# revdotcom/reverb

Hardware: NVIDIA H100
Metric: rtfx_attention_rescoring_30s_chunks (higher is better)
Workload: dtype bf16

## Files before the change

reverb_b200/csrc/attention_tc.cu:

```cuda
#include <cuda.h>
#include <math.h>
#include <stdlib.h>

#include <algorithm>

#include "kernels.h"

namespace rvb {

constexpr int AT_BM = 128;
constexpr int AT_BN = 64;
constexpr int AT_DK = 64;
constexpr int AT_ST = 4;
constexpr int AT_THREADS = 288;
constexpr uint32_t AT_Q_BYTES = AT_BM * AT_DK * 2;
constexpr uint32_t AT_TILE_BYTES = AT_BN * AT_DK * 2;
constexpr uint32_t AT_SMEM_FIXED = AT_Q_BYTES + 2 * AT_ST * AT_TILE_BYTES + 256  + 1024 ;

__device__ __forceinline__ float fast_exp2(float x) {
  float y;
  asm("ex2.approx.ftz.f32 %0, %1;" : "=f"(y) : "f"(x));
  return y;
}

struct AttnTcParams {
  bf16* out;
  long long ldo;
  const float* key_bias;
  const int* k_lens;
  int Tq, Tk, H;
  int chunk;
  int left;
  const uint32_t* key_bits;
  int bits_ld;
  float scale_log2;
};

__global__ void __launch_bounds__(AT_THREADS, 1)
attention_tc_kernel(const __grid_constant__ CUtensorMap tmQ, const __grid_constant__ CUtensorMap tmK,
                    const __grid_constant__ CUtensorMap tmV, const AttnTcParams p) {
  extern __shared__ uint8_t smem_raw[];
  uint8_t* smem = reinterpret_cast<uint8_t*>((reinterpret_cast<uintptr_t>(smem_raw) + 1023) & ~uintptr_t(1023));
  uint8_t* sQ = smem;
  uint8_t* sK = sQ + AT_Q_BYTES;
  uint8_t* sV = sK + AT_ST * AT_TILE_BYTES;
  uint64_t* bars = reinterpret_cast<uint64_t*>(sV + AT_ST * AT_TILE_BYTES);
  uint64_t* q_full = bars;
  uint64_t* k_full = bars + 1;
  uint64_t* k_empty = k_full + AT_ST;
  uint64_t* v_full = k_empty + AT_ST;
  uint64_t* v_empty = v_full + AT_ST;
  static_assert(1 + 4 * AT_ST <= 32, "barrier block is 256 bytes");
  float* s_bias = reinterpret_cast<float*>(bars + 32);

  const int warp = threadIdx.x >> 5, lane = threadIdx.x & 31;
  const int qtile = blockIdx.x, h = blockIdx.y, g = blockIdx.z;
  const int q0 = qtile * AT_BM;
  int klen = p.Tk;
  if (p.k_lens) klen = min(klen, __ldg(p.k_lens + g));
  auto vis_lo = [&](int i) { return (p.chunk > 0 && p.left >= 0) ? max(0, (i / p.chunk - p.left) * p.chunk) : 0; };
  auto vis_hi = [&](int i) { return p.chunk > 0 ? min(klen, (i / p.chunk + 1) * p.chunk) : klen; };
  const int jt0 = vis_lo(q0) / AT_BN;
  const int ntiles = max(0, (vis_hi(q0 + AT_BM - 1) + AT_BN - 1) / AT_BN - jt0);
  const long long krow0 = (long long)g * p.Tk;

  if (threadIdx.x == 0) {
    mbar_init(q_full, 1);
    for (int i = 0; i < AT_ST; ++i) {
      mbar_init(&k_full[i], 1);
      mbar_init(&k_empty[i], 8);
      mbar_init(&v_full[i], 1);
      mbar_init(&v_empty[i], 8);
    }
    fence_barrier_init();
  }
  {
    const float* kb = p.key_bias ? p.key_bias + ((long long)g * p.H + h) * p.Tk : nullptr;
    for (int kk = threadIdx.x; kk < ntiles * AT_BN; kk += AT_THREADS) {
      const int key = jt0 * AT_BN + kk;
      s_bias[kk] = (key < klen) ? (kb ? __ldg(kb + key) * p.scale_log2 : 0.f) : -INFINITY;
    }
  }
  __syncthreads();

  if (warp == 8) {
    if (lane == 0 && ntiles > 0) {
      tma_prefetch_desc(&tmQ);
      tma_prefetch_desc(&tmK);
      tma_prefetch_desc(&tmV);
      mbar_expect_tx(q_full, AT_Q_BYTES);
      tma_load_2d(sQ, &tmQ, q_full, h * AT_DK, (int)((long long)g * p.Tq + q0));
      for (int n = 0; n < ntiles; ++n) {
        const int st = n % AT_ST, ph = ((n / AT_ST) & 1) ^ 1;
        const int krow = (int)(krow0 + (jt0 + n) * AT_BN);
        mbar_wait(&k_empty[st], ph);
        mbar_expect_tx(&k_full[st], AT_TILE_BYTES);
        tma_load_2d(sK + st * AT_TILE_BYTES, &tmK, &k_full[st], h * AT_DK, krow);
        mbar_wait(&v_empty[st], ph);
        mbar_expect_tx(&v_full[st], AT_TILE_BYTES);
        tma_load_2d(sV + st * AT_TILE_BYTES, &tmV, &v_full[st], h * AT_DK, krow);
      }
    }
    return;
  }

  const int wg = warp >> 2, wl = warp & 3;
  const int rloc = wg * 64 + wl * 16 + (lane >> 2);
  const int row[2] = {q0 + rloc, q0 + rloc + 8};
  const int cq = 2 * (lane & 3);
  float o[32];
#pragma unroll
  for (int i = 0; i < 32; ++i) o[i] = 0.f;
  float m_run[2] = {-INFINITY, -INFINITY}, row_sum[2] = {0.f, 0.f};
  if (ntiles > 0) mbar_wait(q_full, 0);
  const uint64_t qdesc = make_sw128_desc(smem_u32(sQ + wg * (AT_Q_BYTES / 2)));
#pragma unroll 1
  for (int j = 0; j < ntiles; ++j) {
    const int st = j % AT_ST, ph = (j / AT_ST) & 1;
    float s[32];
    mbar_wait(&k_full[st], ph);
    {
      const uint64_t kdesc = make_sw128_desc(smem_u32(sK + st * AT_TILE_BYTES));
      wgmma_fence_regs<32>(s);
      wgmma_fence();
#pragma unroll
      for (int k = 0; k < AT_DK / 16; ++k) wgmma_m64n64k16_ss(s, qdesc + 2 * k, kdesc + 2 * k, k != 0);
      wgmma_commit();
      wgmma_wait<0>();
      wgmma_fence_regs<32>(s);
    }
    if (lane == 0) mbar_arrive(&k_empty[st]);
    const int kbase = (jt0 + j) * AT_BN;
    const float* bias = s_bias + j * AT_BN;
    float tmax[2] = {-INFINITY, -INFINITY};
#pragma unroll
    for (int jj = 0; jj < 8; ++jj) {
      const float2 b2 = *reinterpret_cast<const float2*>(bias + 8 * jj + cq);
#pragma unroll
      for (int i = 0; i < 2; ++i) {
        s[4 * jj + 2 * i] = fmaf(s[4 * jj + 2 * i], p.scale_log2, b2.x);
        s[4 * jj + 2 * i + 1] = fmaf(s[4 * jj + 2 * i + 1], p.scale_log2, b2.y);
      }
    }
    if (p.chunk > 0) {
#pragma unroll
      for (int i = 0; i < 2; ++i) {
        const int lo = vis_lo(row[i]) - kbase, hi = vis_hi(row[i]) - kbase;
#pragma unroll
        for (int jj = 0; jj < 8; ++jj)
#pragma unroll
          for (int c = 0; c < 2; ++c) {
            const int col = 8 * jj + cq + c;
            if (col < lo || col >= hi) s[4 * jj + 2 * i + c] = -INFINITY;
          }
      }
    }
    if (p.key_bits) {
#pragma unroll
      for (int i = 0; i < 2; ++i) {
        const uint32_t* mw = p.key_bits + ((long long)g * p.Tq + min(row[i], p.Tq - 1)) * p.bits_ld + (kbase >> 5);
        const uint32_t w0 = __ldg(mw), w1 = __ldg(mw + 1);
#pragma unroll
        for (int jj = 0; jj < 8; ++jj)
#pragma unroll
          for (int c = 0; c < 2; ++c) {
            const int col = 8 * jj + cq + c;
            const uint32_t word = (col < 32) ? w0 : w1;
            if (!((word >> (col & 31)) & 1u)) s[4 * jj + 2 * i + c] = -INFINITY;
          }
      }
    }
#pragma unroll
    for (int jj = 0; jj < 8; ++jj)
#pragma unroll
      for (int i = 0; i < 2; ++i) tmax[i] = fmaxf(tmax[i], fmaxf(s[4 * jj + 2 * i], s[4 * jj + 2 * i + 1]));
#pragma unroll
    for (int i = 0; i < 2; ++i) {
      tmax[i] = fmaxf(tmax[i], __shfl_xor_sync(0xffffffffu, tmax[i], 1));
      tmax[i] = fmaxf(tmax[i], __shfl_xor_sync(0xffffffffu, tmax[i], 2));
    }
    float m_eff[2];
#pragma unroll
    for (int i = 0; i < 2; ++i) {
      const float m_new = fmaxf(m_run[i], tmax[i]);
      const float f = (m_new == -INFINITY || m_run[i] == m_new) ? 1.f : fast_exp2(m_run[i] - m_new);
      m_run[i] = m_new;
      row_sum[i] *= f;
#pragma unroll
      for (int jj = 0; jj < 8; ++jj) {
        o[4 * jj + 2 * i] *= f;
        o[4 * jj + 2 * i + 1] *= f;
      }
      m_eff[i] = (m_new == -INFINITY) ? 0.f : m_new;
    }
    uint32_t pa[16];
#pragma unroll
    for (int jj = 0; jj < 8; ++jj)
#pragma unroll
      for (int i = 0; i < 2; ++i) {
        const uint32_t w = pack_bf16x2(fast_exp2(s[4 * jj + 2 * i] - m_eff[i]), fast_exp2(s[4 * jj + 2 * i + 1] - m_eff[i]));
        const float2 pr = unpack_bf16x2(w);
        row_sum[i] += pr.x + pr.y;
        pa[2 * jj + i] = w;
      }
    mbar_wait(&v_full[st], ph);
    {
      const uint64_t vdesc = make_sw128_desc(smem_u32(sV + st * AT_TILE_BYTES));
      wgmma_fence_regs<32>(o);
      wgmma_fence();
#pragma unroll
      for (int ks = 0; ks < AT_BN / 16; ++ks)
        wgmma_m64n64k16_rs_tb(o, pa + 4 * ks, vdesc + (uint64_t)((ks * 16 * 128) >> 4));
      wgmma_commit();
      wgmma_wait<0>();
      wgmma_fence_regs<32>(o);
    }
    if (lane == 0) mbar_arrive(&v_empty[st]);
  }
#pragma unroll
  for (int i = 0; i < 2; ++i) {
    float sum = row_sum[i];
    sum += __shfl_xor_sync(0xffffffffu, sum, 1);
    sum += __shfl_xor_sync(0xffffffffu, sum, 2);
    const float inv = sum > 0.f ? 1.f / sum : 0.f;
    if (row[i] < p.Tq) {
      bf16* orow = p.out + ((long long)g * p.Tq + row[i]) * p.ldo + h * AT_DK;
#pragma unroll
      for (int jj = 0; jj < 8; ++jj)
        *reinterpret_cast<uint32_t*>(orow + 8 * jj + cq) = pack_bf16x2(o[4 * jj + 2 * i] * inv, o[4 * jj + 2 * i + 1] * inv);
    }
  }
}

__global__ void __launch_bounds__(256)
relpos_prep_kernel(const bf16* __restrict__ k, long long ldk, const bf16* __restrict__ pos, long long ldp,
                   const float* __restrict__ bias_u, const float* __restrict__ bias_v, bf16* __restrict__ kpp,
                   float* __restrict__ cbias, int B, int T, int H, int dk) {
  const long long row = ((long long)blockIdx.x * blockDim.x + threadIdx.x) >> 5;
  const int lane = threadIdx.x & 31;
  if (row >= (long long)B * T) return;
  const int b = (int)(row / T), t = (int)(row - (long long)b * T);
  const int d = H * dk;
  const bf16* kr = k + row * ldk;
  const bf16* pr = pos + (long long)t * ldp;
  bf16* orow = kpp + row * d;
  for (int h = 0; h < H; ++h) {
    float acc = 0.f;
    for (int c = 2 * lane; c < dk; c += 64) {
      const int col = h * dk + c;
      float2 kv = unpack_bf16x2(*reinterpret_cast<const uint32_t*>(kr + col));
      float2 pv = unpack_bf16x2(*reinterpret_cast<const uint32_t*>(pr + col));
// ... 56 lines not shown
                       ((reinterpret_cast<uintptr_t>(pos) & 15) == 0) && ((reinterpret_cast<uintptr_t>(kpp) & 15) == 0) &&
                       ((reinterpret_cast<uintptr_t>(bias_u) & 15) == 0) && ((reinterpret_cast<uintptr_t>(bias_v) & 15) == 0);
  if (aligned && dk == 64)
    relpos_prep_vec_kernel<8><<<grid, 256, 0, stream>>>(k, ldk, pos, ldp, bias_u, bias_v, kpp, cbias, B, T, H);
  else if (aligned && dk == 128)
    relpos_prep_vec_kernel<16><<<grid, 256, 0, stream>>>(k, ldk, pos, ldp, bias_u, bias_v, kpp, cbias, B, T, H);
  else if (aligned && dk == 32)
    relpos_prep_vec_kernel<4><<<grid, 256, 0, stream>>>(k, ldk, pos, ldp, bias_u, bias_v, kpp, cbias, B, T, H);
  else
    relpos_prep_kernel<<<grid, 256, 0, stream>>>(k, ldk, pos, ldp, bias_u, bias_v, kpp, cbias, B, T, H, dk);
  RVB_COUNT_LAUNCH();
  RVB_CHECK_LAUNCH();
  return 0;
}

typedef CUresult (*EncodeTiledFn)(CUtensorMap*, CUtensorMapDataType, cuuint32_t, void*, const cuuint64_t*,
                                  const cuuint64_t*, const cuuint32_t*, const cuuint32_t*, CUtensorMapInterleave,
                                  CUtensorMapSwizzle, CUtensorMapL2promotion, CUtensorMapFloatOOBfill);
static EncodeTiledFn g_encode_att = nullptr;

static int tmap_2d(CUtensorMap* m, const void* base, long long cols, long long rows, long long ld_elems,
                   int box_rows) {
  cuuint64_t dims[2] = {(cuuint64_t)cols, (cuuint64_t)rows};
  cuuint64_t str[1] = {(cuuint64_t)ld_elems * 2};
  cuuint32_t box[2] = {64, (cuuint32_t)box_rows};
  cuuint32_t estr[2] = {1, 1};
  CUresult r = g_encode_att(m, CU_TENSOR_MAP_DATA_TYPE_BFLOAT16, 2, const_cast<void*>(base), dims, str, box, estr,
                            CU_TENSOR_MAP_INTERLEAVE_NONE, CU_TENSOR_MAP_SWIZZLE_128B, CU_TENSOR_MAP_L2_PROMOTION_L2_256B,
                            CU_TENSOR_MAP_FLOAT_OOB_FILL_NONE);
  RVB_REQUIRE(r == CUDA_SUCCESS, "attention: cuTensorMapEncodeTiled failed (%d)", (int)r);
  return 0;
}

int launch_attention_tc(const AttnTcArgs& a, cudaStream_t stream) {
  RVB_REQUIRE(a.dk == AT_DK, "attention_tc: only d_k = 64 is built");
  RVB_REQUIRE(a.ldq % 8 == 0 && a.ldk % 8 == 0 && a.ldv % 8 == 0 && a.ldo % 8 == 0, "attention_tc: ld %% 8 != 0");
  RVB_REQUIRE(((uintptr_t)a.q & 15) == 0 && ((uintptr_t)a.k & 15) == 0 && ((uintptr_t)a.v & 15) == 0 &&
                  ((uintptr_t)a.out & 15) == 0,
              "attention_tc: operands must be 16-byte aligned");
  RVB_REQUIRE((!a.causal && a.chunk <= 0) || a.Tq == a.Tk, "attention_tc: causal / chunk masks need Tq == Tk");
  RVB_REQUIRE(!(a.causal && a.chunk > 0), "attention_tc: causal and chunk mask are exclusive");
  if (a.groups <= 0 || a.Tq <= 0) return 0;
  if (g_encode_att == nullptr) {
    void* fn = nullptr;
    cudaDriverEntryPointQueryResult qres;
    RVB_CHECK_CUDA(cudaGetDriverEntryPoint("cuTensorMapEncodeTiled", &fn, cudaEnableDefault, &qres));
    RVB_REQUIRE(fn != nullptr && qres == cudaDriverEntryPointSuccess, "cuTensorMapEncodeTiled not available");
    g_encode_att = reinterpret_cast<EncodeTiledFn>(fn);
  }
  AttnTcParams p;
  p.out = a.out;
  p.ldo = a.ldo;
  p.key_bias = a.key_bias;
  p.k_lens = a.k_lens;
  p.Tq = a.Tq;
  p.Tk = a.Tk;
  p.H = a.H;
  p.chunk = a.causal ? 1 : (a.chunk > 0 ? a.chunk : 0);
  p.left = a.causal ? -1 : a.left_chunks;
  p.key_bits = a.key_bits;
  p.bits_ld = a.bits_ld;
  RVB_REQUIRE(a.key_bits == nullptr || a.bits_ld >= 2 * ((a.Tk + 63) / 64), "attention_tc: key_bits rows are too short");
  p.scale_log2 = a.scale * 1.4426950408889634f;
  CUtensorMap tmQ, tmK, tmV;
  if (tmap_2d(&tmQ, a.q, (long long)a.H * AT_DK, (long long)a.groups * a.Tq, a.ldq, AT_BM)) return -1;
  if (tmap_2d(&tmK, a.k, (long long)a.H * AT_DK, (long long)a.groups * a.Tk, a.ldk, AT_BN)) return -1;
  if (tmap_2d(&tmV, a.v, (long long)a.H * AT_DK, (long long)a.groups * a.Tk, a.ldv, AT_BN)) return -1;
  dim3 grid((a.Tq + AT_BM - 1) / AT_BM, a.H, a.groups);
  const size_t smem = AT_SMEM_FIXED + (size_t)((a.Tk + AT_BN - 1) / AT_BN) * AT_BN * sizeof(float);
  RVB_REQUIRE(smem <= 227 * 1024, "attention_tc: Tk=%d needs %zu B of shared memory", a.Tk, smem);
  static DynSmemOptIn optin;
  if (optin.ensure(attention_tc_kernel, smem)) return -1;
  attention_tc_kernel<<<grid, AT_THREADS, smem, stream>>>(tmQ, tmK, tmV, p);
  RVB_COUNT_LAUNCH();
  RVB_CHECK_LAUNCH();
  return 0;
}

}
```

include/rvb_b200.h:

```cpp
#ifndef RVB_B200_H_
#define RVB_B200_H_

#if defined(__GNUC__)
#define RVB_API __attribute__((visibility("default")))
#else
#define RVB_API
#endif

#ifdef __cplusplus
extern "C" {
#endif

typedef struct rvb_model rvb_model;

typedef struct rvb_model_config {
  int input_dim;
  int d_model;
  int heads;
  int ffn_dim;
  int num_blocks;
  int cnn_kernel;
  int causal;
  int cnn_layer_norm;
  int num_langs;
// ... 104 lines not shown

typedef struct rvb_aligner rvb_aligner;
RVB_API long long rvb_aligner_workspace_bytes(int U, int total_frames, int want_loglik);
RVB_API rvb_aligner* rvb_aligner_begin(rvb_model* m, const int* h_labels, int U, int total_frames, int V, int blank_id,
                                       int want_loglik, long long budget_bytes, void* stream);
RVB_API int rvb_aligner_push(rvb_aligner* a, const float* d_logp, int n_rows, void* stream);
RVB_API int rvb_aligner_finish(rvb_aligner* a, int* h_frames, int* h_first, int* h_last, int* h_peak, float* h_peak_logp,
                               float* h_score, double* h_loglik, void* stream);
RVB_API void rvb_aligner_abort(rvb_aligner* a);

RVB_API int rvb_gemm_bf16(const void* d_A, const void* d_W, const float* d_bias, int M, int N, int K, int act, int out_mode,
                  float alpha, void* d_out, int ldo, void* stream);
RVB_API int rvb_gemm_bf16_rows(const void* d_A, const void* d_W, const float* d_bias, int M, int N, int K, int act,
                               int out_mode, float alpha, void* d_out, int ldo, const int* d_row_lens, int rows_per_batch,
                               void* stream);
RVB_API int rvb_gemm_bf16x3(const void* d_A, const void* d_W, const float* d_bias, int M, int N, int K, int act, int out_mode,
                            float alpha, void* d_out, int ldo, void* stream);
RVB_API int rvb_f32_to_bf16_pair(const float* d_x, void* d_out, long long rows, int width, void* stream);
RVB_API long long rvb_gemm_logsoftmax_gather_ws_bytes(int M, int N);
RVB_API int rvb_gemm_logsoftmax_gather(const void* d_A, const void* d_W, const float* d_bias, int M, int N, int K,
                                       const int* d_gather, void* d_ws, float* d_out, void* stream);
RVB_API int rvb_layernorm(const float* d_x, const float* d_gamma, const float* d_beta, float eps, int M, int d,
                  void* d_out_bf16, float* d_out_f32, void* stream);
RVB_API int rvb_attention(const void* d_q, const void* d_k, const void* d_v, const void* d_p, const float* d_bias_u,
                  const float* d_bias_v, void* d_out, int ldq, int ldk, int ldv, int ldp, int ldo, int Bq, int Tq, int Tk,
                  int H, int dk, int q_per_kv, const int* d_k_lens, const int* d_q_lens, int causal, float scale,
                  void* stream);
RVB_API int rvb_attention_tc(const void* d_q, const void* d_k, const void* d_v, void* d_out, int ldq, int ldk, int ldv,
                             int ldo, int groups, int Tq, int Tk, int H, int dk, const float* d_key_bias,
                             const int* d_k_lens, int causal, float scale, void* stream);
RVB_API int rvb_attention_tc_chunked(const void* d_q, const void* d_k, const void* d_v, void* d_out, int ldq, int ldk,
                                     int ldv, int ldo, int groups, int Tq, int Tk, int H, int dk, const float* d_key_bias,
                                     const int* d_k_lens, int chunk, int left_chunks, float scale, void* stream);
RVB_API int rvb_relpos_prep(const void* d_k, int ldk, const void* d_pos, int ldp, const float* d_bias_u,
                            const float* d_bias_v, void* d_kpp, float* d_cbias, int B, int T, int H, int dk,
                            void* stream);
RVB_API int rvb_f32_to_bf16(const float* d_x, void* d_out, long long n, void* stream);

#ifdef __cplusplus
}
#endif
#endif
```

reverb_b200/_lib.py:

```python
from __future__ import annotations

import ctypes as C
import os
from typing import Optional

_HERE = os.path.dirname(os.path.abspath(__file__))
LIB_PATH = os.environ.get("RVB_LIB_PATH") or os.path.join(_HERE, "librvb_b200.so")


class ModelConfig(C.Structure):
    _fields_ = [(n, C.c_int) for n in (
        "input_dim", "d_model", "heads", "ffn_dim", "num_blocks", "cnn_kernel", "causal",
        "cnn_layer_norm", "num_langs", "vocab", "dec_heads", "dec_ffn_dim", "dec_blocks", "r_dec_blocks",
        "sos_id", "eos_id", "precision")]


class SegConfig(C.Structure):
    _fields_ = [(n, C.c_int) for n in (
        "sample_rate", "sinc_filters", "sinc_kernel", "sinc_stride", "conv_channels", "conv_kernel", "lstm_hidden",
        "lstm_layers", "linear_dim", "linear_layers", "num_classes")]


class EmbConfig(C.Structure):
    _fields_ = [("sample_rate", C.c_int), ("num_mel_bins", C.c_int), ("m_channels", C.c_int), ("embed_dim", C.c_int),
# ... 32 lines not shown
                                       _vp, _vp, _vp, _vp]),
    "rvb_search_submit": (_i, [_vp, _vp, _vp, _i, _vp, _vp, _i, _i, _i, _i, _vp]),
    "rvb_search_submit_biased": (_i, [_vp, _vp, _vp, _i, _vp, _vp, _i, _i, _i, _i, _vp, _vp]),
    "rvb_context_graph_create": (_vp, [_i, _vp, _vp, _vp, _vp, _vp, _vp, _vp, _i, _i]),
    "rvb_context_graph_destroy": (None, [_vp]),
    "rvb_ctc_prefix_beam_search_biased": (_i, [_vp, _vp, _i, _vp, _i, _i, _i, _i, _i, _vp, _vp, _vp, _vp, _vp, _vp,
                                               _vp]),
    "rvb_rescoring_submit": (_i, [_vp, _i, _vp, _i, _f, _i, _i, _vp, _vp, _vp, _vp, _vp, _vp]),
    "rvb_rescoring_collect": (_i, [_vp, _i, _vp, _vp, _vp]),
    "rvb_ticket_release": (_i, [_vp, _i]),
    "rvb_decoder_step_topk": (_i, [_vp, _vp, _vp, _i, _i, _i, _vp, _i, _vp, _i, _i, _vp, _vp, _vp]),
    "rvb_decoder_cache_begin": (_i, [_vp, _vp, _vp, _i, _i, _i, _i, _vp, _i, _vp]),
    "rvb_decoder_cache_step": (_i, [_vp, _vp, _vp, _i, _vp, _vp, _vp]),
    "rvb_decoder_cache_end": (_i, [_vp]),
    "rvb_decoder_step_logp": (_i, [_vp, _vp, _vp, _i, _i, _i, _vp, _i, _vp, _i, _vp, _vp]),
    "rvb_attention_rescoring": (_i, [_vp, _vp, _vp, _i, _i, _vp, _vp, _i, _i, _vp, _i, _f, _vp, _vp, _vp]),
    "rvb_ctc_force_align": (_i, [_vp, _i, _vp, _i, _i, _vp, _vp, _i, _i, _vp, _vp, _vp, _vp, _vp, _vp, _vp, _vp]),
    "rvb_aligner_workspace_bytes": (_ll, [_i, _i, _i]),
    "rvb_aligner_begin": (_vp, [_vp, _vp, _i, _i, _i, _i, _i, _ll, _vp]),
    "rvb_aligner_push": (_i, [_vp, _vp, _i, _vp]),
    "rvb_aligner_finish": (_i, [_vp, _vp, _vp, _vp, _vp, _vp, _vp, _vp, _vp]),
    "rvb_aligner_abort": (None, [_vp]),
    "rvb_gemm_bf16": (_i, [_vp, _vp, _vp, _i, _i, _i, _i, _i, _f, _vp, _i, _vp]),
    "rvb_gemm_bf16_rows": (_i, [_vp, _vp, _vp, _i, _i, _i, _i, _i, _f, _vp, _i, _vp, _i, _vp]),
    "rvb_gemm_bf16x3": (_i, [_vp, _vp, _vp, _i, _i, _i, _i, _i, _f, _vp, _i, _vp]),
    "rvb_f32_to_bf16_pair": (_i, [_vp, _vp, _ll, _i, _vp]),
    "rvb_gemm_logsoftmax_gather_ws_bytes": (_ll, [_i, _i]),
    "rvb_gemm_logsoftmax_gather": (_i, [_vp, _vp, _vp, _i, _i, _i, _vp, _vp, _vp, _vp]),
    "rvb_layernorm": (_i, [_vp, _vp, _vp, _f, _i, _i, _vp, _vp, _vp]),
    "rvb_attention": (_i, [_vp, _vp, _vp, _vp, _vp, _vp, _vp, _i, _i, _i, _i, _i, _i, _i, _i, _i, _i, _i, _vp, _vp,
                           _i, _f, _vp]),
    "rvb_attention_tc_chunked": (_i, [_vp, _vp, _vp, _vp, _i, _i, _i, _i, _i, _i, _i, _i, _i, _vp, _vp, _i, _i, _f, _vp]),
    "rvb_attention_tc": (_i, [_vp, _vp, _vp, _vp, _i, _i, _i, _i, _i, _i, _i, _i, _i, _vp, _vp, _i, _f, _vp]),
    "rvb_relpos_prep": (_i, [_vp, _i, _vp, _i, _vp, _vp, _vp, _vp, _i, _i, _i, _i, _vp]),
    "rvb_f32_to_bf16": (_i, [_vp, _vp, _ll, _vp]),
    "rvb_seg_create": (_vp, [C.POINTER(SegConfig)]),
    "rvb_seg_set_tensor": (_i, [_vp, C.c_char_p, _vp, _ll]),
    "rvb_seg_finalize": (_i, [_vp]),
    "rvb_seg_destroy": (None, [_vp]),
    "rvb_seg_num_frames": (_i, [_vp, _i]),
    "rvb_seg_forward": (_i, [_vp, _vp, _i, _i, _vp, _vp, _vp]),
    "rvb_emb_create": (_vp, [C.POINTER(EmbConfig)]),
    "rvb_emb_set_tensor": (_i, [_vp, C.c_char_p, _vp, _ll]),
    "rvb_emb_finalize": (_i, [_vp]),
    "rvb_emb_destroy": (None, [_vp]),
    "rvb_emb_num_frames": (_i, [_vp, _i]),
    "rvb_emb_forward": (_i, [_vp, _vp, _i, _i, _vp, _i, _i, _vp, _vp, _vp]),
}

_lib: Optional[C.CDLL] = None


def load() -> C.CDLL:
    global _lib
    if _lib is not None:
        return _lib
    if not os.path.exists(LIB_PATH):
        raise RuntimeError(
            f"{LIB_PATH} is missing: build it with `python -m reverb_b200.build` "
            "(or __graft_entry__.build()). reverb_b200 has no CPU fallback.")
    lib = C.CDLL(LIB_PATH)
    for name, (res, args) in SIGNATURES.items():
        if os.environ.get("RVB_LIB_PATH") and not hasattr(lib, name):
            continue
        fn = getattr(lib, name)
        fn.restype = res
# ... 14 lines not shown
```

reverb_b200/csrc/engine.cu:

```cuda
#include <math.h>
#include <stdarg.h>
#include <stdlib.h>
#include <string.h>

#include <atomic>
#include <map>
#include <string>
#include <vector>

#include "../../include/rvb_b200.h"
#include "kernels.h"

namespace rvb {

static thread_local char g_err[1024] = "";
std::atomic<unsigned long long> g_launch_count{0};
void set_error(const char* fmt, ...) {
  va_list ap;
  va_start(ap, fmt);
  vsnprintf(g_err, sizeof(g_err), fmt, ap);
  va_end(ap);
}
const char* last_error() { return g_err; }

// ... 2149 lines not shown
  a.q = reinterpret_cast<const rvb::bf16*>(d_q);
  a.k = reinterpret_cast<const rvb::bf16*>(d_k);
  a.v = reinterpret_cast<const rvb::bf16*>(d_v);
  a.p = reinterpret_cast<const rvb::bf16*>(d_p);
  a.bias_u = d_bias_u;
  a.bias_v = d_bias_v;
  a.out = reinterpret_cast<rvb::bf16*>(d_out);
  a.ldq = ldq; a.ldk = ldk; a.ldv = ldv; a.ldp = ldp; a.ldo = ldo;
  a.Bq = Bq; a.Tq = Tq; a.Tk = Tk; a.H = H; a.dk = dk;
  a.q_per_kv = q_per_kv;
  a.k_lens = d_k_lens; a.q_lens = d_q_lens;
  a.causal = causal;
  a.scale = scale;
  return rvb::launch_attention(a, (cudaStream_t)stream);
}

RVB_API int rvb_attention_tc(const void* d_q, const void* d_k, const void* d_v, void* d_out, int ldq, int ldk, int ldv,
                             int ldo, int groups, int Tq, int Tk, int H, int dk, const float* d_key_bias,
                             const int* d_k_lens, int causal, float scale, void* stream) {
  rvb::AttnTcArgs a;
  a.q = reinterpret_cast<const rvb::bf16*>(d_q);
  a.k = reinterpret_cast<const rvb::bf16*>(d_k);
  a.v = reinterpret_cast<const rvb::bf16*>(d_v);
  a.out = reinterpret_cast<rvb::bf16*>(d_out);
  a.ldq = ldq; a.ldk = ldk; a.ldv = ldv; a.ldo = ldo;
  a.groups = groups; a.Tq = Tq; a.Tk = Tk; a.H = H; a.dk = dk;
  a.key_bias = d_key_bias;
  a.k_lens = d_k_lens;
  a.causal = causal;
  a.scale = scale;
  return rvb::launch_attention_tc(a, (cudaStream_t)stream);
}

RVB_API int rvb_attention_tc_chunked(const void* d_q, const void* d_k, const void* d_v, void* d_out, int ldq, int ldk,
                                     int ldv, int ldo, int groups, int Tq, int Tk, int H, int dk, const float* d_key_bias,
                                     const int* d_k_lens, int chunk, int left_chunks, float scale, void* stream) {
  rvb::AttnTcArgs a;
  a.q = reinterpret_cast<const rvb::bf16*>(d_q);
  a.k = reinterpret_cast<const rvb::bf16*>(d_k);
  a.v = reinterpret_cast<const rvb::bf16*>(d_v);
  a.out = reinterpret_cast<rvb::bf16*>(d_out);
  a.ldq = ldq; a.ldk = ldk; a.ldv = ldv; a.ldo = ldo;
  a.groups = groups; a.Tq = Tq; a.Tk = Tk; a.H = H; a.dk = dk;
  a.key_bias = d_key_bias;
  a.k_lens = d_k_lens;
  a.chunk = chunk;
  a.left_chunks = left_chunks;
  a.scale = scale;
  return rvb::launch_attention_tc(a, (cudaStream_t)stream);
}

RVB_API int rvb_relpos_prep(const void* d_k, int ldk, const void* d_pos, int ldp, const float* d_bias_u,
                            const float* d_bias_v, void* d_kpp, float* d_cbias, int B, int T, int H, int dk,
                            void* stream) {
  return rvb::launch_relpos_prep(reinterpret_cast<const rvb::bf16*>(d_k), ldk, reinterpret_cast<const rvb::bf16*>(d_pos),
                                 ldp, d_bias_u, d_bias_v, reinterpret_cast<rvb::bf16*>(d_kpp), d_cbias, B, T, H, dk,
                                 (cudaStream_t)stream);
}

RVB_API int rvb_f32_to_bf16(const float* d_x, void* d_out, long long n, void* stream) {
  return rvb::launch_f32_to_bf16(d_x, reinterpret_cast<rvb::bf16*>(d_out), n, (cudaStream_t)stream);
}

}
```

reverb_b200/csrc/kernels.h:

```cpp
#pragma once
#include "common.cuh"

struct rvb_model;
struct rvb_context_graph;

namespace rvb {

int search_side_stream(::rvb_model* m, cudaStream_t* out);

enum GemmAct { ACT_NONE = 0, ACT_RELU = 1, ACT_SILU = 2, ACT_GLU = 3 };
enum GemmOut {
  OUT_BF16 = 0,
  OUT_F32 = 1,
  OUT_RESID_F32 = 2,
  OUT_LSE = 3
};
inline int lse_slabs(int N) { return ((N + 255) / 256) * 2; }

struct GemmArgs {
  const bf16* A = nullptr;
  const bf16* W = nullptr;
  int M = 0, N = 0, K = 0;
  int lda = 0;
  int ldw = 0;
// ... 70 lines not shown
  const bf16* q = nullptr;
  const bf16* k = nullptr;
  const bf16* v = nullptr;
  const bf16* p = nullptr;
  const float* bias_u = nullptr;
  const float* bias_v = nullptr;
  bf16* out = nullptr;
  int ldq = 0, ldk = 0, ldv = 0, ldp = 0, ldo = 0;
  int Bq = 0, Tq = 0, Tk = 0, H = 0, dk = 0;
  int q_per_kv = 1;
  const int* k_lens = nullptr;
  const int* q_lens = nullptr;
  int causal = 0;
  float scale = 1.0f;
};
int launch_attention(const AttnArgs& a, cudaStream_t stream);

struct AttnTcArgs {
  const bf16* q = nullptr;
  const bf16* k = nullptr;
  const bf16* v = nullptr;
  bf16* out = nullptr;
  int ldq = 0, ldk = 0, ldv = 0, ldo = 0;
  int groups = 0, Tq = 0, Tk = 0, H = 0, dk = 0;
  const float* key_bias = nullptr;
  const int* k_lens = nullptr;
  int causal = 0;
  int chunk = 0, left_chunks = -1;
  const uint32_t* key_bits = nullptr;
  int bits_ld = 0;
  float scale = 1.0f;
};
int launch_attention_tc(const AttnTcArgs& a, cudaStream_t stream);
int launch_relpos_prep(const bf16* k, int ldk, const bf16* pos, int ldp, const float* bias_u, const float* bias_v,
                       bf16* kpp, float* cbias, int B, int T, int H, int dk, cudaStream_t stream);

struct AttnF32Args {
  const bf16* q = nullptr;
  const bf16* k = nullptr;
  const bf16* v = nullptr;
  const bf16* p = nullptr;
  const float* bias_u = nullptr;
  const float* bias_v = nullptr;
  bf16* out = nullptr;
  int ldq = 0, ldk = 0, ldv = 0, ldp = 0, ldo = 0;
  int q_lo = 0, k_lo = 0, v_lo = 0, p_lo = 0, o_lo = 0;
  int groups = 0, Tq = 0, Tk = 0, H = 0, dk = 0;
  const int* k_lens = nullptr;
  int chunk = 0, left = -1;
  const int* key_list = nullptr;
  const int* key_list_len = nullptr;
  int key_list_ld = 0;
};
int launch_attention_f32(const AttnF32Args& a, cudaStream_t stream);

int launch_logsoftmax_topk(const float* logits, int ld, int M, int V, int k, float* topk_val, int* topk_idx,
                           float* logp_out , int apply_softmax, cudaStream_t stream);
int launch_ctc_greedy(const int* top1_idx, int idx_stride, const int* lens, int B, int T, int blank, int* out_tokens,
                      int* out_lens, cudaStream_t stream);
struct PrefixBeamWorkspace;
size_t prefix_beam_workspace_bytes(int B, int T, int beam);
int launch_ctc_prefix_beam(const float* topk_val, const int* topk_idx, int k, const int* lens, int B, int T, int beam,
                           int blank, void* workspace, size_t workspace_bytes, int max_len, int* out_tokens,
                           int* out_times, int* out_lens, double* out_scores, int* out_nhyp, cudaStream_t stream);
struct ContextGraphView {
  const int* off = nullptr;
// ... 36 lines not shown
```

Baseline: 11910.

## Overlap QK^T of next tile with PV of current tile in attention kernel

Measured after the change: 11990, median of 6. No clear change (+0.7%).

```diff
diff --git a/reverb_b200/csrc/attention_tc.cu b/reverb_b200/csrc/attention_tc.cu
--- a/reverb_b200/csrc/attention_tc.cu
+++ b/reverb_b200/csrc/attention_tc.cu
@@ -21,6 +21,11 @@
   float y;
   asm("ex2.approx.ftz.f32 %0, %1;" : "=f"(y) : "f"(x));
   return y;
+}
+
+__device__ __forceinline__ void keep_regs16(const uint32_t* r) {
+#pragma unroll
+  for (int i = 0; i < 16; ++i) asm volatile("" ::"r"(r[i]) : "memory");
 }
 
 struct AttnTcParams {
@@ -64,7 +69,8 @@
   const int ntiles = max(0, (vis_hi(q0 + AT_BM - 1) + AT_BN - 1) / AT_BN - jt0);
   const long long krow0 = (long long)g * p.Tk;
 
-  if (threadIdx.x == 0) {
+  const bool producer = threadIdx.x == 8 * 32;
+  if (producer) {
     mbar_init(q_full, 1);
     for (int i = 0; i < AT_ST; ++i) {
       mbar_init(&k_full[i], 1);
@@ -73,6 +79,20 @@
       mbar_init(&v_empty[i], 8);
     }
     fence_barrier_init();
+    if (ntiles > 0) {
+      tma_prefetch_desc(&tmQ);
+      tma_prefetch_desc(&tmK);
+      tma_prefetch_desc(&tmV);
+      mbar_expect_tx(q_full, AT_Q_BYTES);
+      tma_load_2d(sQ, &tmQ, q_full, h * AT_DK, (int)((long long)g * p.Tq + q0));
+      for (int n = 0; n < min(ntiles, AT_ST); ++n) {
+        const int krow = (int)(krow0 + (jt0 + n) * AT_BN);
+        mbar_expect_tx(&k_full[n], AT_TILE_BYTES);
+        tma_load_2d(sK + n * AT_TILE_BYTES, &tmK, &k_full[n], h * AT_DK, krow);
+        mbar_expect_tx(&v_full[n], AT_TILE_BYTES);
+        tma_load_2d(sV + n * AT_TILE_BYTES, &tmV, &v_full[n], h * AT_DK, krow);
+      }
+    }
   }
   {
     const float* kb = p.key_bias ? p.key_bias + ((long long)g * p.H + h) * p.Tk : nullptr;
@@ -84,13 +104,8 @@
   __syncthreads();
 
   if (warp == 8) {
-    if (lane == 0 && ntiles > 0) {
-      tma_prefetch_desc(&tmQ);
-      tma_prefetch_desc(&tmK);
-      tma_prefetch_desc(&tmV);
-      mbar_expect_tx(q_full, AT_Q_BYTES);
-      tma_load_2d(sQ, &tmQ, q_full, h * AT_DK, (int)((long long)g * p.Tq + q0));
-      for (int n = 0; n < ntiles; ++n) {
+    if (producer) {
+      for (int n = AT_ST; n < ntiles; ++n) {
         const int st = n % AT_ST, ph = ((n / AT_ST) & 1) ^ 1;
         const int krow = (int)(krow0 + (jt0 + n) * AT_BN);
         mbar_wait(&k_empty[st], ph);
@@ -114,25 +129,30 @@
   float m_run[2] = {-INFINITY, -INFINITY}, row_sum[2] = {0.f, 0.f};
   if (ntiles > 0) mbar_wait(q_full, 0);
   const uint64_t qdesc = make_sw128_desc(smem_u32(sQ + wg * (AT_Q_BYTES / 2)));
-#pragma unroll 1
-  for (int j = 0; j < ntiles; ++j) {
-    const int st = j % AT_ST, ph = (j / AT_ST) & 1;
-    float s[32];
-    mbar_wait(&k_full[st], ph);
-    {
-      const uint64_t kdesc = make_sw128_desc(smem_u32(sK + st * AT_TILE_BYTES));
-      wgmma_fence_regs<32>(s);
-      wgmma_fence();
-#pragma unroll
-      for (int k = 0; k < AT_DK / 16; ++k) wgmma_m64n64k16_ss(s, qdesc + 2 * k, kdesc + 2 * k, k != 0);
-      wgmma_commit();
-      wgmma_wait<0>();
-      wgmma_fence_regs<32>(s);
-    }
-    if (lane == 0) mbar_arrive(&k_empty[st]);
-    const int kbase = (jt0 + j) * AT_BN;
-    const float* bias = s_bias + j * AT_BN;
-    float tmax[2] = {-INFINITY, -INFINITY};
+
+  auto issue_s = [&](int t, float* s) {
+    const int st = t % AT_ST;
+    mbar_wait(&k_full[st], (t / AT_ST) & 1);
+    const uint64_t kdesc = make_sw128_desc(smem_u32(sK + st * AT_TILE_BYTES));
+    wgmma_fence_regs<32>(s);
+    wgmma_fence();
+#pragma unroll
+    for (int k = 0; k < AT_DK / 16; ++k) wgmma_m64n64k16_ss(s, qdesc + 2 * k, kdesc + 2 * k, k != 0);
+    wgmma_commit();
+  };
+  auto issue_pv = [&](int t, const uint32_t* pa) {
+    const int st = t % AT_ST;
+    mbar_wait(&v_full[st], (t / AT_ST) & 1);
+    const uint64_t vdesc = make_sw128_desc(smem_u32(sV + st * AT_TILE_BYTES));
+    wgmma_fence();
+#pragma unroll
+    for (int ks = 0; ks < AT_BN / 16; ++ks)
+      wgmma_m64n64k16_rs_tb(o, pa + 4 * ks, vdesc + (uint64_t)((ks * 16 * 128) >> 4));
+    wgmma_commit();
+  };
+  auto softmax = [&](int t, float* s, uint32_t* pa, float* f) {
+    const int kbase = (jt0 + t) * AT_BN;
+    const float* bias = s_bias + t * AT_BN;
 #pragma unroll
     for (int jj = 0; jj < 8; ++jj) {
       const float2 b2 = *reinterpret_cast<const float2*>(bias + 8 * jj + cq);
@@ -170,6 +190,7 @@
           }
       }
     }
+    float tmax[2] = {-INFINITY, -INFINITY};
 #pragma unroll
     for (int jj = 0; jj < 8; ++jj)
 #pragma unroll
@@ -183,39 +204,70 @@
 #pragma unroll
     for (int i = 0; i < 2; ++i) {
       const float m_new = fmaxf(m_run[i], tmax[i]);
-      const float f = (m_new == -INFINITY || m_run[i] == m_new) ? 1.f : fast_exp2(m_run[i] - m_new);
+      f[i] = (m_new == -INFINITY || m_run[i] == m_new) ? 1.f : fast_exp2(m_run[i] - m_new);
       m_run[i] = m_new;
-      row_sum[i] *= f;
-#pragma unroll
-      for (int jj = 0; jj < 8; ++jj) {
-        o[4 * jj + 2 * i] *= f;
-        o[4 * jj + 2 * i + 1] *= f;
-      }
       m_eff[i] = (m_new == -INFINITY) ? 0.f : m_new;
     }
-    uint32_t pa[16];
 #pragma unroll
     for (int jj = 0; jj < 8; ++jj)
 #pragma unroll
       for (int i = 0; i < 2; ++i) {
         const uint32_t w = pack_bf16x2(fast_exp2(s[4 * jj + 2 * i] - m_eff[i]), fast_exp2(s[4 * jj + 2 * i + 1] - m_eff[i]));
         const float2 pr = unpack_bf16x2(w);
-        row_sum[i] += pr.x + pr.y;
+        if (jj == 0)
+          row_sum[i] = (i == 1) ? fmaf(row_sum[i], f[i], pr.x + pr.y) : __fmul_rn(row_sum[i], f[i]) + (pr.x + pr.y);
+        else
+          row_sum[i] += pr.x + pr.y;
         pa[2 * jj + i] = w;
       }
-    mbar_wait(&v_full[st], ph);
-    {
-      const uint64_t vdesc = make_sw128_desc(smem_u32(sV + st * AT_TILE_BYTES));
-      wgmma_fence_regs<32>(o);
-      wgmma_fence();
-#pragma unroll
-      for (int ks = 0; ks < AT_BN / 16; ++ks)
-        wgmma_m64n64k16_rs_tb(o, pa + 4 * ks, vdesc + (uint64_t)((ks * 16 * 128) >> 4));
-      wgmma_commit();
-      wgmma_wait<0>();
-      wgmma_fence_regs<32>(o);
-    }
-    if (lane == 0) mbar_arrive(&v_empty[st]);
+  };
+
+  float s[32], f[2];
+  uint32_t pa[16], pb[16];
+  auto step = [&](int j, const uint32_t* pc, uint32_t* pn) {
+    issue_s(j + 1, s);
+    issue_pv(j, pc);
+    wgmma_wait<1>();
+    wgmma_fence_regs<32>(s);
+    if (lane == 0) mbar_arrive(&k_empty[(j + 1) % AT_ST]);
+    softmax(j + 1, s, pn, f);
+    wgmma_wait<0>();
+    wgmma_fence_regs<32>(o);
+    keep_regs16(pc);
+    if (lane == 0) mbar_arrive(&v_empty[j % AT_ST]);
+#pragma unroll
+    for (int i = 0; i < 2; ++i)
+#pragma unroll
+      for (int jj = 0; jj < 8; ++jj) {
+        o[4 * jj + 2 * i] *= f[i];
+        o[4 * jj + 2 * i + 1] *= f[i];
+      }
+    wgmma_fence_regs<32>(o);
+  };
+  auto finish = [&](int j, const uint32_t* pc) {
+    issue_pv(j, pc);
+    wgmma_wait<0>();
+    wgmma_fence_regs<32>(o);
+    keep_regs16(pc);
+  };
+  if (ntiles > 0) {
+    issue_s(0, s);
+    wgmma_wait<0>();
+    wgmma_fence_regs<32>(s);
+    if (lane == 0) mbar_arrive(&k_empty[0]);
+    softmax(0, s, pa, f);
+    int j = 0;
+#pragma unroll 1
+    for (; j + 2 < ntiles; j += 2) {
+      step(j, pa, pb);
+      step(j + 1, pb, pa);
+    }
+    if (j + 1 < ntiles) {
+      step(j, pa, pb);
+      finish(j + 1, pb);
+    } else {
+      finish(j, pa);
+    }
   }
 #pragma unroll
   for (int i = 0; i < 2; ++i) {
```

## Drop TMA producer warp, software-pipeline QK^T with PV, template attention on mask kind

Applied to the files above, without the earlier changes.

After: 11870 before, 12240 after (median of 6 runs). +3.1%, better.

```diff
diff --git a/include/rvb_b200.h b/include/rvb_b200.h
--- a/include/rvb_b200.h
+++ b/include/rvb_b200.h
@@ -160,6 +160,11 @@
 RVB_API int rvb_attention_tc_chunked(const void* d_q, const void* d_k, const void* d_v, void* d_out, int ldq, int ldk,
                                      int ldv, int ldo, int groups, int Tq, int Tk, int H, int dk, const float* d_key_bias,
                                      const int* d_k_lens, int chunk, int left_chunks, float scale, void* stream);
+RVB_API int rvb_attention_tc_bits(const void* d_q, const void* d_k, const void* d_v, void* d_out, int ldq, int ldk,
+                                  int ldv, int ldo, int groups, int Tq, int Tk, int H, int dk, const float* d_key_bias,
+                                  const int* d_k_lens, int causal, const void* d_key_bits, int bits_ld, float scale,
+                                  void* stream);
+RVB_API int rvb_attention_tc_blocks_per_sm(int Tk, int causal, int chunk, int with_key_bits);
 RVB_API int rvb_relpos_prep(const void* d_k, int ldk, const void* d_pos, int ldp, const float* d_bias_u,
                             const float* d_bias_v, void* d_kpp, float* d_cbias, int B, int T, int H, int dk,
                             void* stream);
diff --git a/reverb_b200/_lib.py b/reverb_b200/_lib.py
--- a/reverb_b200/_lib.py
+++ b/reverb_b200/_lib.py
@@ -88,6 +88,9 @@
                            _i, _f, _vp]),
     "rvb_attention_tc_chunked": (_i, [_vp, _vp, _vp, _vp, _i, _i, _i, _i, _i, _i, _i, _i, _i, _vp, _vp, _i, _i, _f, _vp]),
     "rvb_attention_tc": (_i, [_vp, _vp, _vp, _vp, _i, _i, _i, _i, _i, _i, _i, _i, _i, _vp, _vp, _i, _f, _vp]),
+    "rvb_attention_tc_bits": (_i, [_vp, _vp, _vp, _vp, _i, _i, _i, _i, _i, _i, _i, _i, _i, _vp, _vp, _i, _vp, _i, _f,
+                                   _vp]),
+    "rvb_attention_tc_blocks_per_sm": (_i, [_i, _i, _i, _i]),
     "rvb_relpos_prep": (_i, [_vp, _i, _vp, _i, _vp, _vp, _vp, _vp, _i, _i, _i, _i, _vp]),
     "rvb_f32_to_bf16": (_i, [_vp, _vp, _ll, _vp]),
     "rvb_seg_create": (_vp, [C.POINTER(SegConfig)]),
diff --git a/reverb_b200/csrc/attention_tc.cu b/reverb_b200/csrc/attention_tc.cu
--- a/reverb_b200/csrc/attention_tc.cu
+++ b/reverb_b200/csrc/attention_tc.cu
@@ -3,6 +3,7 @@
 #include <stdlib.h>
 
 #include <algorithm>
+#include <type_traits>
 
 #include "kernels.h"
 
@@ -12,7 +13,7 @@
 constexpr int AT_BN = 64;
 constexpr int AT_DK = 64;
 constexpr int AT_ST = 4;
-constexpr int AT_THREADS = 288;
+constexpr int AT_THREADS = 256;
 constexpr uint32_t AT_Q_BYTES = AT_BM * AT_DK * 2;
 constexpr uint32_t AT_TILE_BYTES = AT_BN * AT_DK * 2;
 constexpr uint32_t AT_SMEM_FIXED = AT_Q_BYTES + 2 * AT_ST * AT_TILE_BYTES + 256  + 1024 ;
@@ -36,7 +37,20 @@
   float scale_log2;
 };
 
-__global__ void __launch_bounds__(AT_THREADS, 1)
+enum AttnMask : int {
+  MASK_LENS = 0,
+  MASK_CHUNK = 1,
+  MASK_BITS = 2,
+};
+
+__device__ __forceinline__ void attn_issue_s(float* s, uint64_t qdesc, const uint8_t* k_tile) {
+  const uint64_t kdesc = make_sw128_desc(smem_u32(k_tile));
+#pragma unroll
+  for (int k = 0; k < AT_DK / 16; ++k) wgmma_m64n64k16_ss(s, qdesc + 2 * k, kdesc + 2 * k, k != 0);
+}
+
+template <int MASK>
+__global__ void __launch_bounds__(AT_THREADS, 2)
 attention_tc_kernel(const __grid_constant__ CUtensorMap tmQ, const __grid_constant__ CUtensorMap tmK,
                     const __grid_constant__ CUtensorMap tmV, const AttnTcParams p) {
   extern __shared__ uint8_t smem_raw[];
@@ -58,11 +72,20 @@
   const int q0 = qtile * AT_BM;
   int klen = p.Tk;
   if (p.k_lens) klen = min(klen, __ldg(p.k_lens + g));
-  auto vis_lo = [&](int i) { return (p.chunk > 0 && p.left >= 0) ? max(0, (i / p.chunk - p.left) * p.chunk) : 0; };
-  auto vis_hi = [&](int i) { return p.chunk > 0 ? min(klen, (i / p.chunk + 1) * p.chunk) : klen; };
+  const bool chunked = MASK == MASK_CHUNK || (MASK == MASK_BITS && p.chunk > 0);
+  auto vis_lo = [&](int i) { return (chunked && p.left >= 0) ? max(0, (i / p.chunk - p.left) * p.chunk) : 0; };
+  auto vis_hi = [&](int i) { return chunked ? min(klen, (i / p.chunk + 1) * p.chunk) : klen; };
   const int jt0 = vis_lo(q0) / AT_BN;
   const int ntiles = max(0, (vis_hi(q0 + AT_BM - 1) + AT_BN - 1) / AT_BN - jt0);
   const long long krow0 = (long long)g * p.Tk;
+  auto load_tile = [&](int n) {
+    const int st = n % AT_ST;
+    const int krow = (int)(krow0 + (jt0 + n) * AT_BN);
+    mbar_expect_tx(&k_full[st], AT_TILE_BYTES);
+    tma_load_2d(sK + st * AT_TILE_BYTES, &tmK, &k_full[st], h * AT_DK, krow);
+    mbar_expect_tx(&v_full[st], AT_TILE_BYTES);
+    tma_load_2d(sV + st * AT_TILE_BYTES, &tmV, &v_full[st], h * AT_DK, krow);
+  };
 
   if (threadIdx.x == 0) {
     mbar_init(q_full, 1);
@@ -73,6 +96,11 @@
       mbar_init(&v_empty[i], 8);
     }
     fence_barrier_init();
+    if (ntiles > 0) {
+      mbar_expect_tx(q_full, AT_Q_BYTES);
+      tma_load_2d(sQ, &tmQ, q_full, h * AT_DK, (int)((long long)g * p.Tq + q0));
+      for (int n = 0; n < min(ntiles, AT_ST); ++n) load_tile(n);
+    }
   }
   {
     const float* kb = p.key_bias ? p.key_bias + ((long long)g * p.H + h) * p.Tk : nullptr;
@@ -83,27 +111,6 @@
   }
   __syncthreads();
 
-  if (warp == 8) {
-    if (lane == 0 && ntiles > 0) {
-      tma_prefetch_desc(&tmQ);
-      tma_prefetch_desc(&tmK);
-      tma_prefetch_desc(&tmV);
-      mbar_expect_tx(q_full, AT_Q_BYTES);
-      tma_load_2d(sQ, &tmQ, q_full, h * AT_DK, (int)((long long)g * p.Tq + q0));
-      for (int n = 0; n < ntiles; ++n) {
-        const int st = n % AT_ST, ph = ((n / AT_ST) & 1) ^ 1;
-        const int krow = (int)(krow0 + (jt0 + n) * AT_BN);
-        mbar_wait(&k_empty[st], ph);
-        mbar_expect_tx(&k_full[st], AT_TILE_BYTES);
-        tma_load_2d(sK + st * AT_TILE_BYTES, &tmK, &k_full[st], h * AT_DK, krow);
-        mbar_wait(&v_empty[st], ph);
-        mbar_expect_tx(&v_full[st], AT_TILE_BYTES);
-        tma_load_2d(sV + st * AT_TILE_BYTES, &tmV, &v_full[st], h * AT_DK, krow);
-      }
-    }
-    return;
-  }
-
   const int wg = warp >> 2, wl = warp & 3;
   const int rloc = wg * 64 + wl * 16 + (lane >> 2);
   const int row[2] = {q0 + rloc, q0 + rloc + 8};
@@ -112,24 +119,29 @@
 #pragma unroll
   for (int i = 0; i < 32; ++i) o[i] = 0.f;
   float m_run[2] = {-INFINITY, -INFINITY}, row_sum[2] = {0.f, 0.f};
-  if (ntiles > 0) mbar_wait(q_full, 0);
   const uint64_t qdesc = make_sw128_desc(smem_u32(sQ + wg * (AT_Q_BYTES / 2)));
-#pragma unroll 1
-  for (int j = 0; j < ntiles; ++j) {
+  float s[32];
+  if (ntiles > 0) {
+    mbar_wait(q_full, 0);
+    mbar_wait(&k_full[0], 0);
+    wgmma_fence_regs<32>(s);
+    wgmma_fence();
+    attn_issue_s(s, qdesc, sK);
+    wgmma_commit();
+    wgmma_wait<0>();
+    wgmma_fence_regs<32>(s);
+    if (lane == 0) mbar_arrive(&k_empty[0]);
+  }
+  auto tile = [&](const int j, auto next_tag) {
+    constexpr bool next = decltype(next_tag)::value;
     const int st = j % AT_ST, ph = (j / AT_ST) & 1;
-    float s[32];
-    mbar_wait(&k_full[st], ph);
-    {
-      const uint64_t kdesc = make_sw128_desc(smem_u32(sK + st * AT_TILE_BYTES));
-      wgmma_fence_regs<32>(s);
-      wgmma_fence();
-#pragma unroll
-      for (int k = 0; k < AT_DK / 16; ++k) wgmma_m64n64k16_ss(s, qdesc + 2 * k, kdesc + 2 * k, k != 0);
-      wgmma_commit();
-      wgmma_wait<0>();
-      wgmma_fence_regs<32>(s);
-    }
-    if (lane == 0) mbar_arrive(&k_empty[st]);
+    if (threadIdx.x == 0 && j > 0 && j - 1 + AT_ST < ntiles) {
+      const int n = j - 1 + AT_ST, ph_free = ((n / AT_ST) & 1) ^ 1;
+      mbar_wait(&k_empty[n % AT_ST], ph_free);
+      mbar_wait(&v_empty[n % AT_ST], ph_free);
+      load_tile(n);
+    }
+    __syncwarp();
     const int kbase = (jt0 + j) * AT_BN;
     const float* bias = s_bias + j * AT_BN;
     float tmax[2] = {-INFINITY, -INFINITY};
@@ -142,7 +154,7 @@
         s[4 * jj + 2 * i + 1] = fmaf(s[4 * jj + 2 * i + 1], p.scale_log2, b2.y);
       }
     }
-    if (p.chunk > 0) {
+    if (chunked) {
 #pragma unroll
       for (int i = 0; i < 2; ++i) {
         const int lo = vis_lo(row[i]) - kbase, hi = vis_hi(row[i]) - kbase;
@@ -155,7 +167,7 @@
           }
       }
     }
-    if (p.key_bits) {
+    if (MASK == MASK_BITS) {
 #pragma unroll
       for (int i = 0; i < 2; ++i) {
         const uint32_t* mw = p.key_bits + ((long long)g * p.Tq + min(row[i], p.Tq - 1)) * p.bits_ld + (kbase >> 5);
@@ -203,20 +215,31 @@
         row_sum[i] += pr.x + pr.y;
         pa[2 * jj + i] = w;
       }
+    const int st1 = (j + 1) % AT_ST;
     mbar_wait(&v_full[st], ph);
+    if (next) mbar_wait(&k_full[st1], ((j + 1) / AT_ST) & 1);
     {
       const uint64_t vdesc = make_sw128_desc(smem_u32(sV + st * AT_TILE_BYTES));
       wgmma_fence_regs<32>(o);
+      wgmma_fence_regs<32>(s);
       wgmma_fence();
 #pragma unroll
       for (int ks = 0; ks < AT_BN / 16; ++ks)
         wgmma_m64n64k16_rs_tb(o, pa + 4 * ks, vdesc + (uint64_t)((ks * 16 * 128) >> 4));
+      if (next) attn_issue_s(s, qdesc, sK + st1 * AT_TILE_BYTES);
       wgmma_commit();
       wgmma_wait<0>();
       wgmma_fence_regs<32>(o);
-    }
-    if (lane == 0) mbar_arrive(&v_empty[st]);
-  }
+      wgmma_fence_regs<32>(s);
+    }
+    if (lane == 0) {
+      mbar_arrive(&v_empty[st]);
+      if (next) mbar_arrive(&k_empty[st1]);
+    }
+  };
+#pragma unroll 1
+  for (int j = 0; j + 1 < ntiles; ++j) tile(j, std::true_type());
+  if (ntiles > 0) tile(ntiles - 1, std::false_type());
 #pragma unroll
   for (int i = 0; i < 2; ++i) {
     float sum = row_sum[i];
@@ -339,6 +362,42 @@
   return 0;
 }
 
+static int attn_mask_kind(bool chunk_or_causal, bool key_bits) {
+  return key_bits ? MASK_BITS : chunk_or_causal ? MASK_CHUNK : MASK_LENS;
+}
+
+static size_t attn_smem_bytes(int Tk) { return AT_SMEM_FIXED + (size_t)((Tk + AT_BN - 1) / AT_BN) * AT_BN * sizeof(float); }
+
+template <int MASK>
+static int attn_opt_in(size_t smem) {
+  static DynSmemOptIn optin;
+  return optin.ensure(attention_tc_kernel<MASK>, smem);
+}
+
+template <int MASK>
+static int attn_launch(dim3 grid, size_t smem, cudaStream_t stream, const CUtensorMap& tmQ, const CUtensorMap& tmK,
+                       const CUtensorMap& tmV, const AttnTcParams& p) {
+  if (attn_opt_in<MASK>(smem)) return -1;
+  attention_tc_kernel<MASK><<<grid, AT_THREADS, smem, stream>>>(tmQ, tmK, tmV, p);
+  return 0;
+}
+
+template <int MASK>
+static int attn_blocks_per_sm(size_t smem, int* blocks) {
+  if (attn_opt_in<MASK>(smem)) return -1;
+  RVB_CHECK_CUDA(cudaOccupancyMaxActiveBlocksPerMultiprocessor(blocks, attention_tc_kernel<MASK>, AT_THREADS, smem));
+  return 0;
+}
+
+int attention_tc_blocks_per_sm(int Tk, bool chunk_or_causal, bool key_bits, int* blocks) {
+  const size_t smem = attn_smem_bytes(Tk);
+  switch (attn_mask_kind(chunk_or_causal, key_bits)) {
+    case MASK_LENS: return attn_blocks_per_sm<MASK_LENS>(smem, blocks);
+    case MASK_CHUNK: return attn_blocks_per_sm<MASK_CHUNK>(smem, blocks);
+    default: return attn_blocks_per_sm<MASK_BITS>(smem, blocks);
+  }
+}
+
 int launch_attention_tc(const AttnTcArgs& a, cudaStream_t stream) {
   RVB_REQUIRE(a.dk == AT_DK, "attention_tc: only d_k = 64 is built");
   RVB_REQUIRE(a.ldq % 8 == 0 && a.ldk % 8 == 0 && a.ldv % 8 == 0 && a.ldo % 8 == 0, "attention_tc: ld %% 8 != 0");
@@ -374,11 +433,15 @@
   if (tmap_2d(&tmK, a.k, (long long)a.H * AT_DK, (long long)a.groups * a.Tk, a.ldk, AT_BN)) return -1;
   if (tmap_2d(&tmV, a.v, (long long)a.H * AT_DK, (long long)a.groups * a.Tk, a.ldv, AT_BN)) return -1;
   dim3 grid((a.Tq + AT_BM - 1) / AT_BM, a.H, a.groups);
-  const size_t smem = AT_SMEM_FIXED + (size_t)((a.Tk + AT_BN - 1) / AT_BN) * AT_BN * sizeof(float);
+  const size_t smem = attn_smem_bytes(a.Tk);
   RVB_REQUIRE(smem <= 227 * 1024, "attention_tc: Tk=%d needs %zu B of shared memory", a.Tk, smem);
-  static DynSmemOptIn optin;
-  if (optin.ensure(attention_tc_kernel, smem)) return -1;
-  attention_tc_kernel<<<grid, AT_THREADS, smem, stream>>>(tmQ, tmK, tmV, p);
+  int rc;
+  switch (attn_mask_kind(a.causal || a.chunk > 0, a.key_bits != nullptr)) {
+    case MASK_LENS: rc = attn_launch<MASK_LENS>(grid, smem, stream, tmQ, tmK, tmV, p); break;
+    case MASK_CHUNK: rc = attn_launch<MASK_CHUNK>(grid, smem, stream, tmQ, tmK, tmV, p); break;
+    default: rc = attn_launch<MASK_BITS>(grid, smem, stream, tmQ, tmK, tmV, p); break;
+  }
+  if (rc) return rc;
   RVB_COUNT_LAUNCH();
   RVB_CHECK_LAUNCH();
   return 0;
diff --git a/reverb_b200/csrc/engine.cu b/reverb_b200/csrc/engine.cu
--- a/reverb_b200/csrc/engine.cu
+++ b/reverb_b200/csrc/engine.cu
@@ -2205,6 +2205,33 @@
   return rvb::launch_attention_tc(a, (cudaStream_t)stream);
 }
 
+RVB_API int rvb_attention_tc_bits(const void* d_q, const void* d_k, const void* d_v, void* d_out, int ldq, int ldk,
+                                  int ldv, int ldo, int groups, int Tq, int Tk, int H, int dk, const float* d_key_bias,
+                                  const int* d_k_lens, int causal, const void* d_key_bits, int bits_ld, float scale,
+                                  void* stream) {
+  rvb::AttnTcArgs a;
+  a.q = reinterpret_cast<const rvb::bf16*>(d_q);
+  a.k = reinterpret_cast<const rvb::bf16*>(d_k);
+  a.v = reinterpret_cast<const rvb::bf16*>(d_v);
+  a.out = reinterpret_cast<rvb::bf16*>(d_out);
+  a.ldq = ldq; a.ldk = ldk; a.ldv = ldv; a.ldo = ldo;
+  a.groups = groups; a.Tq = Tq; a.Tk = Tk; a.H = H; a.dk = dk;
+  a.key_bias = d_key_bias;
+  a.k_lens = d_k_lens;
+  a.causal = causal;
+  a.key_bits = reinterpret_cast<const uint32_t*>(d_key_bits);
+  a.bits_ld = bits_ld;
+  a.scale = scale;
+  RVB_REQUIRE(d_key_bits != nullptr, "rvb_attention_tc_bits: d_key_bits is null");
+  return rvb::launch_attention_tc(a, (cudaStream_t)stream);
+}
+
+RVB_API int rvb_attention_tc_blocks_per_sm(int Tk, int causal, int chunk, int with_key_bits) {
+  int blocks = 0;
+  if (rvb::attention_tc_blocks_per_sm(Tk, causal || chunk > 0, with_key_bits != 0, &blocks)) return -1;
+  return blocks;
+}
+
 RVB_API int rvb_attention_tc_chunked(const void* d_q, const void* d_k, const void* d_v, void* d_out, int ldq, int ldk,
                                      int ldv, int ldo, int groups, int Tq, int Tk, int H, int dk, const float* d_key_bias,
                                      const int* d_k_lens, int chunk, int left_chunks, float scale, void* stream) {
diff --git a/reverb_b200/csrc/kernels.h b/reverb_b200/csrc/kernels.h
--- a/reverb_b200/csrc/kernels.h
+++ b/reverb_b200/csrc/kernels.h
@@ -126,6 +126,7 @@
   float scale = 1.0f;
 };
 int launch_attention_tc(const AttnTcArgs& a, cudaStream_t stream);
+int attention_tc_blocks_per_sm(int Tk, bool chunk_or_causal, bool key_bits, int* blocks);
 int launch_relpos_prep(const bf16* k, int ldk, const bf16* pos, int ldp, const float* bias_u, const float* bias_v,
                        bf16* kpp, float* cbias, int B, int T, int H, int dk, cudaStream_t stream);
 
```
